# appyjain21/pilottai

Hardware: AMD Instinct MI355X
Metric: completed agent-tasks/sec (whole node) + p50 task latency, 64 concurrent workers (higher is better)
Workload: dtype bf16

## Files before the change

csrc/ops/gemm_stream.hip:

```cpp
#include "common.h"
#include "packed_epi.h"

#include <algorithm>
#include <type_traits>

namespace pa {
namespace sg {

using pk::EP_PLAIN;
using pk::EP_SILU;
using pk::EP_RESID;
using pk::EP_ROPEPERM;
using pk::EP_ROPEKV;
using pk::store_quad;

struct Args {
  bf16* y;
  const bf16* x;
  const bf16* wp;
  const bf16* resid;
  float* ws;
  int* counters;
  int* err;
  int M, N, K, ldx, ldy, ldr;
  int S, RG, G;
  int KSW;
  int epi;
  float eps;
  const float* ss_in;
  float* ss_out;
  float* ss_zero;
  bf16* q_out;
  bf16* k_cache;
  bf16* v_cache;
  const int* positions;
  const int* slots;
  const float* cos_sin;
  int H, KV;
  int rel;
  unsigned long long* stamps;
};

typedef __attribute__((address_space(1))) int gi32;

template <int N>
__device__ __forceinline__ void wait_lgkm() {
  static_assert(N >= 0 && N < 16, "lgkmcnt is 4 bits");
  __builtin_amdgcn_s_waitcnt(0xF | (7 << 4) | (N << 8) | (3 << 14));
}

__device__ __forceinline__ void raw_barrier() {
  asm volatile("" ::: "memory");
  __builtin_amdgcn_s_barrier();
  asm volatile("" ::: "memory");
}

__device__ __forceinline__ void group_barrier(int* arrive, int n, int* err, int rel) {
  __syncthreads();
  if (threadIdx.x == 0) {
    if (rel) {
      __builtin_amdgcn_fence(__ATOMIC_RELEASE, "agent");
      asm volatile("s_waitcnt vmcnt(0)" ::: "memory");
    }
    const int tk = __hip_atomic_fetch_add((gi32*)arrive, 1, __ATOMIC_RELAXED, __HIP_MEMORY_SCOPE_AGENT);
    if (tk != n - 1) {
      const unsigned long long t0 = __builtin_amdgcn_s_memrealtime();
      while (__hip_atomic_load((gi32*)arrive, __ATOMIC_RELAXED, __HIP_MEMORY_SCOPE_AGENT) < n) {
        __builtin_amdgcn_s_sleep(1);
        if (__builtin_amdgcn_s_memrealtime() - t0 > 100000000ull) {
          __hip_atomic_store((gi32*)err, 1, __ATOMIC_RELAXED, __HIP_MEMORY_SCOPE_AGENT);
          break;
        }
      }
    }
    __builtin_amdgcn_fence(__ATOMIC_ACQUIRE, "agent");
    asm volatile("s_waitcnt vmcnt(0)" ::: "memory");
  }
  __syncthreads();
}

template <int EPI>
__device__ __forceinline__ float epi_quad(const Args& A, int m, int tile, int cq, f32x4 v, f32x4 v2) {
  return store_quad<EPI>(A, m, tile, cq, v, v2);
}

struct Pre {
  float rs;
  bf16x4 rv;
  f32x4 c, sn;
  int slot;
};

__device__ __forceinline__ Pre preload(const Args& A, int m, int tile, int cq) {
  Pre p;
  p.rs = 1.f;
  p.slot = -1;
  p.c = f32x4{1.f, 1.f, 1.f, 1.f};
  p.sn = f32x4{0.f, 0.f, 0.f, 0.f};
  if (m >= A.M) return p;
  if (A.ss_in) p.rs = rsqrtf(A.ss_in[m] * (1.f / (float)A.K) + A.eps);
  if (A.epi == EP_RESID) {
    p.rv = *reinterpret_cast<const bf16x4*>(A.resid + (size_t)m * A.ldr + tile * 16 + cq);
  } else if (A.epi == EP_ROPEKV) {
    const int hh = tile >> 3;
    const int d = 16 * ((tile & 7) >> 1) + cq;
    if (hh < A.H + A.KV) {
      const float* cs = A.cos_sin + (size_t)A.positions[m] * 128;
      p.c = *reinterpret_cast<const f32x4*>(cs + d);
      p.sn = *reinterpret_cast<const f32x4*>(cs + 64 + d);
    }
    if (hh >= A.H) p.slot = A.slots[m];
  }
  return p;
}

__device__ __forceinline__ float epi_pre(const Args& A, int m, int tile, int cq, f32x4 v, f32x4 v2, const Pre& p) {
  if (A.epi == EP_SILU) return store_quad<EP_SILU>(A, m, tile, cq, v, v2);
  if (A.epi == EP_PLAIN) return store_quad<EP_PLAIN>(A, m, tile, cq, v, v2);
  if (A.epi == EP_ROPEPERM) return store_quad<EP_ROPEPERM>(A, m, tile, cq, v, v2);
  if (A.epi == EP_RESID) {
    bf16x4 o;
    float sq = 0.f;
#pragma unroll
    for (int r = 0; r < 4; ++r) {
      o[r] = (bf16)(v[r] + (float)p.rv[r]);
      const float f = (float)o[r];
      sq = fmaf(f, f, sq);
    }
    *reinterpret_cast<bf16x4*>(A.y + (size_t)m * A.ldy + tile * 16 + cq) = o;
    return sq;
  }
  const int hh = tile >> 3;
  const int d = 16 * ((tile & 7) >> 1) + cq;
  f32x4 o1 = v, o2 = v2;
  if (hh < A.H + A.KV) {
    o1 = v * p.c - v2 * p.sn;
    o2 = v2 * p.c + v * p.sn;
  }
  bf16x4 b1, b2;
#pragma unroll
  for (int r = 0; r < 4; ++r) {
    b1[r] = (bf16)o1[r];
    b2[r] = (bf16)o2[r];
  }
  if (hh < A.H) {
    bf16* dst = A.q_out + ((size_t)m * A.H + hh) * 128;
    *reinterpret_cast<bf16x4*>(dst + d) = b1;
    *reinterpret_cast<bf16x4*>(dst + d + 64) = b2;
  } else if (p.slot >= 0) {
    const int blk = p.slot >> 4, off = p.slot & 15;
    if (hh < A.H + A.KV) {
      bf16* page = A.k_cache + ((size_t)blk * A.KV + (hh - A.H)) * 128 * 16;
      *reinterpret_cast<bf16x4*>(page + ((size_t)(d >> 3) * 16 + off) * 8 + (d & 7)) = b1;
      *reinterpret_cast<bf16x4*>(page + ((size_t)((d + 64) >> 3) * 16 + off) * 8 + (d & 7)) = b2;
    } else {
      bf16* page = A.v_cache + ((size_t)blk * A.KV + (hh - A.H - A.KV)) * 128 * 16 + off;
#pragma unroll
      for (int r = 0; r < 4; ++r) {
        page[(size_t)(d + r) * 16] = b1[r];
        page[(size_t)(d + 64 + r) * 16] = b2[r];
      }
    }
  }
  return 0.f;
}

template <int MG, int TPW, int WT, int WK, int D>
__global__ __launch_bounds__(WT * WK * 64) void stream_gemm_kernel(const Args A) {
  constexpr int W = WT * WK, NTH = W * 64;
  constexpr int MT = 16 * MG;
  constexpr int CT = WT * TPW;
  constexpr int KW = 2, KC = 2 * WK;
  constexpr int XCH = WK * MT * 128;
  constexpr int XU = WK * MT * 8;
  constexpr int LX = (XU + NTH - 1) / NTH;
  static_assert(D == 2 || D == 4 || D == 8 || D == 16, "even ring depth (LDS slot = chunk & 1)");
  __shared__ __attribute__((aligned(1024))) char smem[2 * XCH + MT * 4 + 16];
  float* rsq = reinterpret_cast<float*>(smem + 2 * XCH);

  const int lane = threadIdx.x & 63;
  const int wid = __builtin_amdgcn_readfirstlane(threadIdx.x >> 6);
  const int wt = wid % WT, wk = wid / WT;
  const int nwg = gridDim.x, bid = blockIdx.x;
  const int q8 = nwg >> 3, r8 = nwg & 7, xcd = bid & 7;
  const int work = (xcd < r8 ? xcd * (q8 + 1) : r8 * (q8 + 1) + (xcd - r8) * q8) + (bid >> 3);
  const int rg = work % A.RG;
  const int s = (work / A.RG) % A.S;
  const int grp = work / (A.RG * A.S);
  const int gid = grp * A.RG + rg;
  const int row0 = rg * MT;
  const int t0 = grp * CT;
  const int KS = A.K >> 5;
  const int kb0 = s * A.KSW;
  const int nch = A.KSW / KC;
  const int rot = (A.rel & 2) ? (work * 5) % nch : 0;

  auto stamp = [&](int i) {
    if (A.stamps && threadIdx.x == 0) A.stamps[(size_t)bid * 8 + i] = __builtin_amdgcn_s_memrealtime();
  };
  stamp(0);
  if (A.ss_zero && bid == 0)
    for (int i = threadIdx.x; i < A.M; i += NTH) A.ss_zero[i] = 0.f;
  for (int i = threadIdx.x; i < MT; i += NTH) rsq[i] = 0.f;

  const bf16x8* wsrc[TPW];
#pragma unroll
  for (int j = 0; j < TPW; ++j)
    wsrc[j] = reinterpret_cast<const bf16x8*>(A.wp + ((size_t)(t0 + wt * TPW + j) * KS + kb0 + wk * KW) * 512) + lane;
  const bf16* xsrc[LX];
  int xdst[LX];
#pragma unroll
  for (int i = 0; i < LX; ++i) {
    const int e = (threadIdx.x + i * NTH) % XU;
    const int h = e / (MT * 8), r = (e >> 3) % MT, u = e & 7;
    const int gr = min(row0 + r, A.M - 1);
    xsrc[i] = A.x + (size_t)gr * A.ldx + kb0 * 32 + h * 64 + u * 8;
    xdst[i] = h * MT * 128 + r * 128 + ((u ^ ((r >> 1) & 7)) << 4);
  }

  bf16x8 wr[D][KW][TPW];
  bf16x8 xr[D][LX];
  f32x4 acc[MG][TPW];
#pragma unroll
  for (int i = 0; i < MG; ++i)
#pragma unroll
    for (int j = 0; j < TPW; ++j) acc[i][j] = f32x4{0.f, 0.f, 0.f, 0.f};

  auto issue = [&](int c0, int d) {
    const int c = rot ? (c0 + rot) % nch : c0;
    __builtin_amdgcn_sched_barrier(0);
#pragma unroll
    for (int i = 0; i < LX; ++i) xr[d][i] = *reinterpret_cast<const bf16x8*>(xsrc[i] + (size_t)c * KC * 32);
#pragma unroll
    for (int i = 0; i < KW; ++i)
#pragma unroll
      for (int j = 0; j < TPW; ++j) wr[d][i][j] = __builtin_nontemporal_load(wsrc[j] + (size_t)(c * KC + i) * 64);
    __builtin_amdgcn_sched_barrier(0);
  };
  auto consume = [&](int d, int slot) {
    char* st = smem + slot * XCH;
#pragma unroll
    for (int i = 0; i < LX; ++i) *reinterpret_cast<bf16x8*>(st + xdst[i]) = xr[d][i];
    wait_lgkm<0>();
    raw_barrier();
#pragma unroll
    for (int i = 0; i < KW; ++i) {
      const int kk = wk * KW + i;
      const int hb = (kk >> 1) * MT * 128, ks = kk & 1;
      bf16x8 xf[MG];
#pragma unroll
      for (int mg = 0; mg < MG; ++mg) {
        const int row = mg * 16 + (lane & 15);
        const int u = 4 * ks + (lane >> 4);
        xf[mg] = *reinterpret_cast<const bf16x8*>(st + hb + row * 128 + ((u ^ ((row >> 1) & 7)) << 4));
      }
#pragma unroll
      for (int mg = 0; mg < MG; ++mg)
#pragma unroll
        for (int j = 0; j < TPW; ++j)
          acc[mg][j] = __builtin_amdgcn_mfma_f32_16x16x32_bf16(wr[d][i][j], xf[mg], acc[mg][j], 0, 0, 0);
    }
  };

#pragma unroll
  for (int d = 0; d < D; ++d) issue(d, d);
  int c = 0;
  for (; c + D < nch; c += D) {
#pragma unroll
    for (int d = 0; d < D; ++d) {
      consume(d, d & 1);
      if (c == 0 && d == 0) stamp(1);
      issue(c + d + D, d);
    }
  }
#pragma unroll
  for (int d = 0; d < D; ++d) {
    consume(d, d & 1);
    if (c == 0 && d == 0) stamp(1);
  }
  stamp(2);

  const bool pair = A.epi == EP_SILU || A.epi == EP_ROPEKV;
  const float inv_k = 1.f / (float)A.K;
  const int g = lane >> 4, cl = lane & 15;
  auto epi_any = [&](int m, int tile, f32x4 v, f32x4 v2) -> float {
    switch (A.epi) {
      case EP_PLAIN: return epi_quad<EP_PLAIN>(A, m, tile, 4 * g, v, v2);
      case EP_SILU: return epi_quad<EP_SILU>(A, m, tile, 4 * g, v, v2);
      case EP_RESID: return epi_quad<EP_RESID>(A, m, tile, 4 * g, v, v2);
      case EP_ROPEPERM: return epi_quad<EP_ROPEPERM>(A, m, tile, 4 * g, v, v2);
      default: return epi_quad<EP_ROPEKV>(A, m, tile, 4 * g, v, v2);
    }
  };
  auto row_stat = [&](int mg, int m, float sq) {
    sq += __shfl_xor(sq, 16, 64);
    sq += __shfl_xor(sq, 32, 64);
    if (g == 0 && m < A.M) atomicAdd(rsq + mg * 16 + cl, sq);
  };
  auto flush_row_stats = [&]() {
    __syncthreads();
    if (A.ss_out)
      for (int i = threadIdx.x; i < MT; i += NTH) {
        const float v = rsq[i];
        if (v != 0.f && row0 + i < A.M) atomicAdd(A.ss_out + row0 + i, v);
      }
  };

  if (A.S * WK == 1 && (!pair || TPW % 2 == 0)) {
#pragma unroll
    for (int mg = 0; mg < MG; ++mg) {
      const int m = row0 + mg * 16 + cl;
      float sq = 0.f;
      if (m < A.M) {
        const float rs = A.ss_in ? rsqrtf(A.ss_in[m] * inv_k + A.eps) : 1.f;
        if (pair) {
#pragma unroll
          for (int j = 0; j + 1 < TPW; j += 2) epi_any(m, t0 + wt * TPW + j, acc[mg][j] * rs, acc[mg][j + 1] * rs);
        } else {
#pragma unroll
          for (int j = 0; j < TPW; ++j) sq += epi_any(m, t0 + wt * TPW + j, acc[mg][j] * rs, acc[mg][j]);
        }
      }
      if (A.ss_out) row_stat(mg, m, sq);
    }
    flush_row_stats();
    stamp(3);
    stamp(4);
    return;
  }

  const int TU = pair ? CT / 2 : CT;
  const int U = TU * MG;
  const int u0 = s + A.S * wid;
  Pre pre0{};
  if (u0 < U) {
    const int tl = pair ? 2 * (u0 / MG) : u0 / MG;
    pre0 = preload(A, row0 + (u0 % MG) * 16 + cl, t0 + tl, 4 * g);
  }

  const int SV = A.S * WK;
  float* gslab = A.ws + (size_t)gid * SV * CT * MG * 256;
  {
    const __amdgpu_buffer_rsrc_t rs =
        __builtin_amdgcn_make_buffer_rsrc(gslab, 0, SV * CT * MG * 1024, 0x00020000);
    const int sv = s * WK + wk;
#pragma unroll
    for (int j = 0; j < TPW; ++j)
#pragma unroll
      for (int mg = 0; mg < MG; ++mg) {
        const int f = (wt * TPW + j) * MG + mg;
        __builtin_amdgcn_raw_buffer_store_b128(__builtin_bit_cast(u32x4, acc[mg][j]), rs,
                                               ((sv * CT * MG + f) * 64 + lane) * 16, 0, 16);
      }
  }
  asm volatile("s_waitcnt vmcnt(0)" ::: "memory");
  int* ctr = A.counters + 2 * gid;
  group_barrier(ctr, A.S, A.err, A.rel & 1);
  stamp(3);

  const __amdgpu_buffer_rsrc_t ra = __builtin_amdgcn_make_buffer_rsrc(gslab, 0, SV * CT * MG * 1024, 0x00020000);
  for (int u = s + A.S * wid; u < U; u += A.S * W) {
    const int tu = u / MG, mg = u % MG;
    const int tl = pair ? 2 * tu : tu;
    const int f = tl * MG + mg;
    f32x4 v = f32x4{0.f, 0.f, 0.f, 0.f}, v2 = f32x4{0.f, 0.f, 0.f, 0.f};
    auto gather = [&](auto two) {
      constexpr bool TWO = decltype(two)::value;
      for (int p0 = 0; p0 < SV; p0 += 8) {
        f32x4 ta[8], tb[8];
#pragma unroll
        for (int q = 0; q < 8; ++q) {
          const int p = min(p0 + q, SV - 1);
          ta[q] = __builtin_bit_cast(f32x4, __builtin_amdgcn_raw_buffer_load_b128(ra, ((p * CT * MG + f) * 64 + lane) * 16, 0, 16));
          if constexpr (TWO)
            tb[q] = __builtin_bit_cast(
                f32x4, __builtin_amdgcn_raw_buffer_load_b128(ra, ((p * CT * MG + f + MG) * 64 + lane) * 16, 0, 16));
        }
#pragma unroll
        for (int q = 0; q < 8; ++q) {
          const float keep = p0 + q < SV ? 1.f : 0.f;
          v += ta[q] * keep;
          if constexpr (TWO) v2 += tb[q] * keep;
        }
      }
    };
    if (pair) gather(std::true_type{});
    else gather(std::false_type{});
    const int m = row0 + mg * 16 + cl;
    float sq = 0.f;
    if (m < A.M) {
      if (u == u0) {
        sq = epi_pre(A, m, t0 + tl, 4 * g, v * pre0.rs, v2 * pre0.rs, pre0);
      } else {
        const float rs = A.ss_in ? rsqrtf(A.ss_in[m] * inv_k + A.eps) : 1.f;
        sq = epi_any(m, t0 + tl, v * rs, v2 * rs);
      }
    }
    if (A.ss_out) row_stat(mg, m, sq);
  }
  flush_row_stats();
  stamp(4);
  if (threadIdx.x == 0) {
    const int left = __hip_atomic_fetch_add((gi32*)(ctr + 1), 1, __ATOMIC_RELAXED, __HIP_MEMORY_SCOPE_AGENT);
    if (left == A.S - 1) {
      __hip_atomic_store((gi32*)ctr, 0, __ATOMIC_RELAXED, __HIP_MEMORY_SCOPE_AGENT);
      __hip_atomic_store((gi32*)(ctr + 1), 0, __ATOMIC_RELAXED, __HIP_MEMORY_SCOPE_AGENT);
    }
  }
}

struct Shape {
  int tpw, wt, wk;
};
static const Shape kShapes[] = {
    {1, 4, 1}, {2, 4, 1}, {3, 4, 1}, {4, 4, 1}, {1, 4, 2}, {2, 2, 2}, {3, 2, 2},
    {1, 6, 1}, {2, 6, 1}, {2, 7, 1}, {2, 8, 1}, {1, 8, 1},
};

template <int MG, int TPW, int WT, int WK>
static bool launch_d(const Args& a, int D, int grid, hipStream_t st) {
  switch (D) {
    case 2: hipLaunchKernelGGL((stream_gemm_kernel<MG, TPW, WT, WK, 2>), dim3(grid), dim3(WT * WK * 64), 0, st, a); return true;
    case 4: hipLaunchKernelGGL((stream_gemm_kernel<MG, TPW, WT, WK, 4>), dim3(grid), dim3(WT * WK * 64), 0, st, a); return true;
    case 8: hipLaunchKernelGGL((stream_gemm_kernel<MG, TPW, WT, WK, 8>), dim3(grid), dim3(WT * WK * 64), 0, st, a); return true;
    case 16: hipLaunchKernelGGL((stream_gemm_kernel<MG, TPW, WT, WK, 16>), dim3(grid), dim3(WT * WK * 64), 0, st, a); return true;
    default: return false;
  }
}

template <int MG>
static bool launch_mg(const Args& a, int tpw, int wt, int wk, int D, int grid, hipStream_t st) {
#define PA_SG(T_, W_, K_) \
  if (tpw == T_ && wt == W_ && wk == K_) return launch_d<MG, T_, W_, K_>(a, D, grid, st);
  PA_SG(1, 4, 1) PA_SG(2, 4, 1) PA_SG(3, 4, 1) PA_SG(4, 4, 1) PA_SG(1, 4, 2) PA_SG(2, 2, 2) PA_SG(3, 2, 2)
  PA_SG(1, 6, 1) PA_SG(2, 6, 1) PA_SG(2, 7, 1) PA_SG(2, 8, 1) PA_SG(1, 8, 1)
#undef PA_SG
  return false;
}

struct Plan {
  int mg, rg, tpw, wt, wk, S, D;
};

static int num_cus() {
  static int n = 0;
  if (n == 0) {
    int dev = 0, v = 0;
    if (hipGetDevice(&dev) == hipSuccess && hipDeviceGetAttribute(&v, hipDeviceAttributeMultiprocessorCount, dev) == hipSuccess && v > 0)
      n = v;
    else
      n = 256;
  }
  return n;
}

static bool plan_ok(const Plan& p, int M, int N, int K, int epi) {
  const int tiles = N / 16, KS = K / 32;
  const int CT = p.tpw * p.wt;
  if (p.mg != 2 && p.mg != 4 && p.mg != 8) return false;
  if (p.rg < 1 || 16 * p.mg * p.rg < M || 16 * p.mg * (p.rg - 1) >= M) return false;
  if (tiles % CT) return false;
  if ((epi == EP_SILU || epi == EP_ROPEKV) && CT % 2) return false;
  if (p.S < 1 || KS % p.S) return false;
  const int KC = 2 * p.wk;
  const int ksw = KS / p.S;
  if (ksw % KC) return false;
  const int nch = ksw / KC;
  if (nch < p.D || nch % p.D) return false;
  if (p.S > 1 && (tiles / CT) * p.rg * p.S > num_cus()) return false;
  return true;
}

static Plan plan_default(int M, int N, int K, int epi) {
  Plan p{};
  p.mg = M <= 32 ? 2 : (M <= 64 ? 4 : 8);
  p.rg = (M + 16 * p.mg - 1) / (16 * p.mg);
  const int tiles = N / 16;
  const bool two = p.rg > 1;
  p.wk = 1;
  p.D = 4;
  if (tiles == 1792) {
    p.tpw = 2; p.wt = 7; p.S = two ? 1 : 2;
  } else if (K >= 8192) {
    p.tpw = 2; p.wt = 4; p.S = two ? 4 : 8;
  } else if (tiles == 384) {
    if (two) { p.tpw = 3; p.wt = 4; p.S = 4; }
    else { p.tpw = 3; p.wt = 2; p.wk = 2; p.S = 4; }
  } else if (tiles == 256) {
    if (two) { p.tpw = 2; p.wt = 4; p.S = 4; }
    else { p.tpw = 1; p.wt = 4; p.wk = 2; p.S = 4; }
  } else if (tiles % 16 == 0 && tiles >= 4096) {
    p.tpw = 4; p.wt = 4; p.S = 1;
  } else {
    p.tpw = 1; p.wt = 4; p.S = 1; p.D = 2;
  }
  if (!plan_ok(p, M, N, K, epi)) {
    p.tpw = 1; p.wt = 4; p.wk = 1; p.S = 1; p.D = 2;
  }
  return p;
}

}
}

extern "C" long long pa_stream_gemm_ws_floats(int M, int N, int K, int mg, int rg, int tpw, int wt, int wk, int S) {
  (void)M; (void)K;
  const long long CT = (long long)tpw * wt, G = N / 16 / CT;
  return G * rg * S * wk * CT * mg * 256;
}

extern "C" void pa_stream_gemm_plan(int M, int N, int K, int epi, int* plan) {
  const pa::sg::Plan p = pa::sg::plan_default(M, N, K, epi);
  plan[0] = p.mg; plan[1] = p.rg; plan[2] = p.tpw; plan[3] = p.wt; plan[4] = p.wk; plan[5] = p.S; plan[6] = p.D;
}

extern "C" int pa_stream_gemm(void* y, const void* x, const void* wp, const void* resid, float* ws,
                              long long ws_floats, int* counters, int n_counters, int* err, int M, int N, int K,
                              int ldx, int ldy, int ldr, int epi, const float* ss_in, float* ss_out, float* ss_zero,
                              float eps, const int* plan, void* q_out, void* k_cache, void* v_cache,
                              const int* positions, const int* slots, const float* cos_sin, int H, int KV, int rel,
                              unsigned long long* stamps, hipStream_t st) {
  using namespace pa::sg;
  if (M <= 0) return 0;
  if (M > 256 || K % 64 != 0 || N % 16 != 0 || epi < 0 || epi > 4) return 1;
  if (epi == EP_RESID && !resid) return 1;
  if (ss_out && epi != EP_RESID) return 1;
  if (epi == EP_ROPEKV && (!q_out || !k_cache || !v_cache || !positions || !slots || !cos_sin ||
                           N != (H + 2 * KV) * 128))
    return 1;
  Plan p = plan_default(M, N, K, epi);
  if (plan && plan[0] > 0 && plan[1] > 0 && plan[2] > 0 && plan[3] > 0 && plan[4] > 0 && plan[5] > 0 && plan[6] > 0)
    p = Plan{plan[0], plan[1], plan[2], plan[3], plan[4], plan[5], plan[6]};
  if (!plan_ok(p, M, N, K, epi)) return 1;
  const int CT = p.tpw * p.wt;
  const int G = N / 16 / CT;
  const int groups = G * p.rg;
  if (!ws || !counters || !err || n_counters < 2 * groups) return 1;
  const bool direct = p.S * p.wk == 1 && (!(epi == EP_SILU || epi == EP_ROPEKV) || p.tpw % 2 == 0);
  if (!direct && pa_stream_gemm_ws_floats(M, N, K, p.mg, p.rg, p.tpw, p.wt, p.wk, p.S) > ws_floats) return 1;
  const int grid = groups * p.S;
  Args a{(pa::bf16*)y, (const pa::bf16*)x, (const pa::bf16*)wp, (const pa::bf16*)resid, ws, counters, err,
         M, N, K, ldx, ldy, ldr, p.S, p.rg, G, K / 32 / p.S, epi, eps, ss_in, ss_out, ss_zero,
         (pa::bf16*)q_out, (pa::bf16*)k_cache, (pa::bf16*)v_cache, positions, slots, cos_sin, H, KV, rel,
         stamps};
  bool ok = false;
  switch (p.mg) {
    case 2: ok = launch_mg<2>(a, p.tpw, p.wt, p.wk, p.D, grid, st); break;
    case 4: ok = launch_mg<4>(a, p.tpw, p.wt, p.wk, p.D, grid, st); break;
    case 8: ok = launch_mg<8>(a, p.tpw, p.wt, p.wk, p.D, grid, st); break;
    default: ok = false;
  }
  if (!ok) return 1;
  return (int)hipGetLastError() == 0 ? 0 : -2;
}
```

pilottai_amd/models/llama.py:

```python
from __future__ import annotations

import math
import os
from dataclasses import dataclass, field
from typing import Dict, List, Optional

import torch
import torch.nn.functional as F

from pilottai_amd import ops
from pilottai_amd.ops import reference as ref
from pilottai_amd.parallel.comm import TPGroup


@dataclass
class LlamaConfig:
    name: str = "llama-3-8b"
    vocab_size: int = 128256
    hidden_size: int = 4096
    intermediate_size: int = 14336
    num_layers: int = 32
    num_heads: int = 32
    num_kv_heads: int = 8
    head_dim: int = 128
    rope_theta: float = 500000.0
    rope_scaling: Optional[dict] = None
    rms_eps: float = 1e-5
    max_position: int = 8192
    tie_embeddings: bool = False
    init_std: float = 0.02

    @property
    def gqa_group(self) -> int:
        return self.num_heads // self.num_kv_heads

    def num_params(self) -> int:
        d, f, v = self.hidden_size, self.intermediate_size, self.vocab_size
        qkv = d * (self.num_heads + 2 * self.num_kv_heads) * self.head_dim
        per_layer = qkv + self.num_heads * self.head_dim * d + 3 * d * f + 2 * d
        return self.num_layers * per_layer + v * d * (1 if self.tie_embeddings else 2) + d


PRESETS: Dict[str, LlamaConfig] = {
    "llama-3-8b": LlamaConfig(),
    "llama-3-70b": LlamaConfig(name="llama-3-70b", hidden_size=8192, intermediate_size=28672,
                               num_layers=80, num_heads=64, num_kv_heads=8),
    "llama-3.1-8b": LlamaConfig(name="llama-3.1-8b", max_position=131072,
                                rope_scaling={"factor": 8.0, "low_freq_factor": 1.0,
                                              "high_freq_factor": 4.0,
                                              "original_max_position_embeddings": 8192}),
    "tiny": LlamaConfig(name="tiny", hidden_size=512, intermediate_size=1024, num_layers=2,
                        num_heads=4, num_kv_heads=1, max_position=4096),
    "tiny-gqa4": LlamaConfig(name="tiny-gqa4", hidden_size=1024, intermediate_size=2048,
                             num_layers=2, num_heads=8, num_kv_heads=2, max_position=4096),
    "tiny-kv8": LlamaConfig(name="tiny-kv8", hidden_size=1024, intermediate_size=2048, num_layers=2,
                            num_heads=16, num_kv_heads=8, max_position=4096),
    "llama-3-8b-2l": LlamaConfig(name="llama-3-8b-2l", num_layers=2, max_position=4096),
    "llama-3-70b-1l": LlamaConfig(name="llama-3-70b-1l", hidden_size=8192, intermediate_size=28672,
                                  num_layers=1, num_heads=64, num_kv_heads=8, max_position=4096),
    "llama-3-70b-2l": LlamaConfig(name="llama-3-70b-2l", hidden_size=8192, intermediate_size=28672,
                                  num_layers=2, num_heads=64, num_kv_heads=8, max_position=4096),
}


def get_config(name_or_cfg) -> LlamaConfig:
    if isinstance(name_or_cfg, LlamaConfig):
        return name_or_cfg
    key = str(name_or_cfg).lower()
    if key not in PRESETS:
        raise ValueError(f"unknown model {name_or_cfg!r}; known: {sorted(PRESETS)}")
    return PRESETS[key]


@dataclass
class StepMeta:
    input_ids: torch.Tensor
    positions: torch.Tensor
    slots: torch.Tensor
    q_start: torch.Tensor
    q_len: torch.Tensor
    ctx_len: torch.Tensor
    block_table: torch.Tensor
    items: torch.Tensor
    n_items: torch.Tensor
    att_counters: torch.Tensor
    logit_rows: torch.Tensor
    num_seqs: int = 0
    part_size: Optional[torch.Tensor] = None


class KVCache:

    def __init__(self, num_layers: int, num_blocks: int, kv_heads: int, device, dtype=torch.bfloat16,
                 block_size: int = 16):
        self.num_blocks = num_blocks
        self.block_size = block_size
        self.k = torch.zeros(num_layers, num_blocks, kv_heads, 16, block_size, 8, dtype=dtype, device=device)
        self.v = torch.zeros(num_layers, num_blocks, kv_heads, 128, block_size, dtype=dtype, device=device)

    @staticmethod
    def bytes_per_block(num_layers: int, kv_heads: int, block_size: int = 16) -> int:
        return 2 * num_layers * kv_heads * block_size * 128 * 2


DENSE_KINDS = ("wqkv", "wo", "w13", "w2")


class LlamaModel:
    DECODE_FUSED_MAX_T = 16
    MID_MAX_T = 256
    PREFILL_MAX_T = 1 << 30
    PF_MIDRANGE = frozenset({"gate_up"})
    DEC_QKV_MAX_T = 0
    ATT_DECODE_WAVES = int(os.environ.get("PILOTTAI_ATT_DECODE_WAVES", "8"))
    ATT_MID_WAVES = int(os.environ.get("PILOTTAI_ATT_MID_WAVES", "4"))
    PF_CFG = {
        "qkv": [(80, "mid", {}), (1280, "pf", {"bn": 128, "variant": 3}),
                (2048, "pf", {"bn": 192, "variant": 3}), (3840, "pf", {"bn": 256, "variant": 3}),
                (1 << 30, "pf", {"bn": 192, "variant": 3})],
        "o": [(128, "mid", {}), (1 << 30, "pf", {"bn": 128, "variant": 3})],
        "gate_up": [(128, "mid", {}), (256, "pf", {"bn": 128, "variant": 3}),
                    (1 << 30, "pf", {"bn": 256, "variant": 3})],
        "down": [(128, "mid", {}), (512, "pf", {"bn": 128, "variant": 3}),
                 (1 << 30, "pf", {"bn": 256, "variant": 3})],
    }
    STREAM_CFG: Dict[str, list] = {
        "qkv": [(32, (1, 1, 4, 1, 2, 4))],
        "o": [(64, (1, 1, 4, 1, 4, 4)), (128, (1, 1, 4, 1, 4, 2))],
        "down": [(32, (1, 1, 4, 1, 4, 4)), (128, (1, 2, 4, 1, 8, 2)), (256, (2, 2, 8, 1, 7, 2))],
    }
    STREAM_NK: Dict[str, tuple] = {"qkv": (6144, 4096), "o": (4096, 4096), "gate_up": (28672, 4096),
                                   "down": (4096, 14336), "lm_head": (128256, 4096)}
    LM_HEAD_STREAM: list = [(32, (1, 3, 4, 1, 1, 2)), (64, (1, 4, 4, 1, 1, 2)), (128, (1, 2, 8, 1, 1, 2))]
    MID_CFG = {
        "qkv": [(32, 1, 2, 2), (64, 1, 2, 1), (128, 2, 2, 1), (256, 4, 2, 1), (1 << 30, 4, 4, 1)],
        "o": [(32, 1, 2, 4), (64, 1, 2, 2), (128, 2, 2, 2), (256, 2, 2, 1), (1 << 30, 4, 2, 1)],
        "gate_up": [(32, 1, 4, 1), (64, 2, 4, 1), (128, 4, 4, 1), (256, 8, 4, 1), (1 << 30, 8, 4, 1)],
        "down": [(32, 1, 2, 4), (64, 2, 2, 4), (128, 2, 2, 2), (256, 4, 2, 2), (1 << 30, 4, 4, 2)],
    }

    def __init__(self, cfg: LlamaConfig, device, dtype=torch.bfloat16, tp: Optional[TPGroup] = None,
                 seed: int = 0, weights_path: Optional[str] = None, decode_pack: Optional[bool] = None,
                 keep_dense: Optional[bool] = None, weight_quant: Optional[str] = None, fp8_decode: bool = True):
        self.cfg = cfg
        self.device = torch.device(device)
        self.dtype = dtype
        self.tp = tp or TPGroup.single()
        if weight_quant not in (None, "fp8"):
            raise ValueError(f"unknown weight_quant {weight_quant!r} (None or 'fp8')")
        if weight_quant and self.tp.size > 1:
            raise ValueError("weight_quant='fp8' needs tensor-parallel size 1: per-channel scales of "
                             "row-parallel shards are not designed yet")
        if weight_quant and decode_pack is False:
            raise ValueError("weight_quant='fp8' lives on the packed weight copies: it cannot be combined "
                             "with decode_pack=False (EngineConfig.decode_fused=False)")
        self.weight_quant = weight_quant
        self.fp8_decode = bool(fp8_decode) and weight_quant == "fp8"
        ov = os.environ.get("PILOTTAI_ROUTING_JSON")
        if ov:
            import json

            for table, rows in json.loads(ov).items():
                if table == "PF_MIDRANGE":
                    self.PF_MIDRANGE = frozenset(rows)
                    continue
                if table not in ("STREAM_CFG", "MID_CFG", "PF_CFG"):
                    raise ValueError(f"PILOTTAI_ROUTING_JSON: unknown table {table!r}")
                merged = dict(getattr(self, table))
                for kind, r in rows.items():
                    merged[kind] = [tuple(x) if table == "MID_CFG" else
                                    (x[0], tuple(x[1])) if table == "STREAM_CFG" else (x[0], x[1], dict(x[2]))
                                    for x in r]
                setattr(self, table, merged)
        ts = self.tp.size
        if cfg.num_heads % ts or cfg.num_kv_heads % ts or cfg.intermediate_size % ts or cfg.vocab_size % ts:
            raise ValueError(f"{cfg.name} is not divisible by tensor-parallel size {ts}")
        self.h_local = cfg.num_heads // ts
        self.kv_local = cfg.num_kv_heads // ts
        self.f_local = cfg.intermediate_size // ts
        self.v_local = cfg.vocab_size // ts
        self.vocab_offset = self.tp.rank * self.v_local
        self.scale = 1.0 / math.sqrt(cfg.head_dim)
        self.cos_sin = ref.rope_cos_sin(cfg.max_position, cfg.head_dim, cfg.rope_theta,
                                        cfg.rope_scaling).to(self.device)
        if weights_path:
            self._load_hf(weights_path)
        else:
            self._init_random(seed)
        self.decode_packed = False
        self.keep_dense = (self.device.type != "cuda") if keep_dense is None else bool(keep_dense)
        if decode_pack is None:
            decode_pack = self._pack_fits()
        if weight_quant:
            self._check_quant_fits(decode_pack)
        if decode_pack:
            self._pack_decode_weights()

    def _pack_fits(self) -> bool:
        if self.device.type != "cuda":
            return True
        total = torch.cuda.get_device_properties(self.device).total_memory
        extra = self._fp8_copy_bytes() if self.fp8_decode else 0
        if self.keep_dense:
            return 2 * self.weight_bytes() + extra <= 0.45 * total
        return self.weight_bytes() + extra <= 0.7 * total

    def _fp8_copy_bytes(self) -> int:
        n = 0
        for L in self.layers:
            for k in DENSE_KINDS:
                w = L[k]
                n += w.numel() + 4 * w.shape[0]
        return n

    def _check_quant_fits(self, decode_pack: bool):
        if decode_pack or self.device.type != "cuda":
            return
        total = torch.cuda.get_device_properties(self.device).total_memory
        base, extra = self.weight_bytes(), (self._fp8_copy_bytes() if self.fp8_decode else 0)
        hint = (": build the model with fp8_decode=False (the same quantised model on the bf16 decode kernels)"
                if self.fp8_decode else "")
        raise ValueError(f"weight_quant={self.weight_quant!r}: {base / 1e9:.2f} GB of bf16 weights"
                         f"{' (kept row-major copy doubles them)' if self.keep_dense else ''} + "
                         f"{extra / 1e9:.2f} GB of FP8 decode copies do not fit beside the KV cache on a "
                         f"{total / 1e9:.0f} GB device{hint}")

    def _pack_decode_weights(self):
        for L in self.layers:
            if self.weight_quant == "fp8":
                self._pack_layer_fp8(L)
            else:
                L["wqkv_p"] = ops.pack_decode_qkv_rope(L["wqkv"] * L["ln1"][None, :])
                L["wo_p"] = ops.pack_decode_weight(L["wo"])
                L["w13_p"] = ops.pack_decode_gate_up(L["w13"] * L["ln2"][None, :])
                L["w2_p"] = ops.pack_decode_weight(L["w2"])
            if not self.keep_dense:
                for k in DENSE_KINDS:
                    del L[k]
        self.lm_head_p = ops.pack_decode_weight(self.lm_head)
        if not self.keep_dense and self.lm_head is not self.embed and self.lm_head.shape[0] % 256 == 0:
            self.lm_head = None
        if self.device.type == "cuda":
            ops.decode_workspace(self.device)
            ops.mid_workspace(self.device)
            ops.prefill_workspace(self.device)
            ops.stream_workspace(self.device)
        self._ss = torch.zeros(2, 1 << 15, dtype=torch.float32, device=self.device)
        self.decode_packed = True

    def _pack_layer_fp8(self, L: Dict[str, torch.Tensor]):
        plan = (("wqkv", "ln1", ops.pack_decode_qkv_rope, ops.pack_decode_qkv_rope_fp8),
                ("wo", None, ops.pack_decode_weight, ops.pack_decode_weight_fp8),
                ("w13", "ln2", ops.pack_decode_gate_up, ops.pack_decode_gate_up_fp8),
                ("w2", None, ops.pack_decode_weight, ops.pack_decode_weight_fp8))
        for kind, ln, pack, pack8 in plan:
            w = L[kind] * L[ln][None, :] if ln else L[kind]
            q, s = ops.quantize_fp8_rows(w)
            deq = ops.dequantize_fp8_rows(q, s, self.dtype)
            del w
            L[kind + "_p"] = pack(deq)
            if self.fp8_decode:
                L[kind + "_p8"], L[kind + "_s8"] = pack8((q, s))
            if self.keep_dense:
                L[kind] = (deq.float() / L[ln].float()[None, :]).to(self.dtype) if ln else deq
            del q, s, deq

    def dense(self, L: Dict[str, torch.Tensor], kind: str) -> torch.Tensor:
        w = L.get(kind)
        if w is not None:
            return w
        if kind == "wqkv":
            return (ops.unpack_decode_qkv_rope(L["wqkv_p"]).float() / L["ln1"].float()[None, :]).to(self.dtype)
        if kind == "w13":
            return (ops.unpack_decode_gate_up(L["w13_p"]).float() / L["ln2"].float()[None, :]).to(self.dtype)
        return ops.unpack_decode_weight(L[{"wo": "wo_p", "w2": "w2_p"}[kind]])

    def dense_lm_head(self) -> torch.Tensor:
        return self.lm_head if self.lm_head is not None else ops.unpack_decode_weight(self.lm_head_p)

    def _dense_needed(self, T: int) -> bool:
        return not self.decode_packed or T > max(self.MID_MAX_T, self.PREFILL_MAX_T)

    def _init_random(self, seed: int):
        cfg, dev, dt = self.cfg, self.device, self.dtype
        C = cfg.num_kv_heads
        ts, r = self.tp.size, self.tp.rank
        if C % ts:
            raise ValueError(f"TP size {ts} must divide num_kv_heads={C}")
        mine = range(r * C // ts, (r + 1) * C // ts)
        std, d, hd = cfg.init_std, cfg.hidden_size, cfg.head_dim

        def chunk(tag: int, j: int, *shape):
            g = torch.Generator(device=dev)
            g.manual_seed((seed * 1_000_003 + tag * 7919 + j) & 0x7FFFFFFF)
            t = torch.empty(*shape, dtype=dt, device=dev)
            t.normal_(0.0, std, generator=g)
            return t

        def rows(tag, total_rows, cols):
            return torch.cat([chunk(tag, j, total_rows // C, cols) for j in mine], 0)

        def colsplit(tag, rows_, total_cols):
            return torch.cat([chunk(tag, j, rows_, total_cols // C) for j in mine], 1)

        self.embed = rows(1, cfg.vocab_size, d)
        self.layers: List[Dict[str, torch.Tensor]] = []
        for li in range(cfg.num_layers):
            t = 100 + 10 * li
            q = rows(t + 0, cfg.num_heads * hd, d)
            k = rows(t + 1, cfg.num_kv_heads * hd, d)
            v = rows(t + 2, cfg.num_kv_heads * hd, d)
            gate = rows(t + 4, cfg.intermediate_size, d)
            up = rows(t + 5, cfg.intermediate_size, d)
            self.layers.append({
                "ln1": torch.ones(d, dtype=dt, device=dev),
                "wqkv": torch.cat([q, k, v], 0),
                "wo": colsplit(t + 3, d, cfg.num_heads * hd),
                "ln2": torch.ones(d, dtype=dt, device=dev),
                "w13": torch.cat([gate, up], 0),
                "w2": colsplit(t + 6, d, cfg.intermediate_size),
            })
            del q, k, v, gate, up
        self.norm = torch.ones(d, dtype=dt, device=dev)
        self.lm_head = self.embed if cfg.tie_embeddings else rows(2, cfg.vocab_size, d)

    def _load_hf(self, path: str):
        from safetensors import safe_open

        cfg, dev, dt = self.cfg, self.device, self.dtype
        files = sorted(f for f in os.listdir(path) if f.endswith(".safetensors"))
        tensors: Dict[str, torch.Tensor] = {}
        for f in files:
            with safe_open(os.path.join(path, f), framework="pt") as fh:
                for k in fh.keys():
                    tensors[k] = fh.get_tensor(k)
        r, ts, hd = self.tp.rank, self.tp.size, cfg.head_dim

        def rows(t, n):
            return t.chunk(ts, dim=0)[r] if ts > 1 else t

        def cols(t):
            return t.chunk(ts, dim=1)[r] if ts > 1 else t

        def get(k):
            return tensors[k].to(dt)

        self.embed = rows(get("model.embed_tokens.weight"), 0).to(dev)
        self.layers = []
        for i in range(cfg.num_layers):
            p = f"model.layers.{i}."
            q = rows(get(p + "self_attn.q_proj.weight"), 0)
            k = rows(get(p + "self_attn.k_proj.weight"), 0)
            v = rows(get(p + "self_attn.v_proj.weight"), 0)
            gate = rows(get(p + "mlp.gate_proj.weight"), 0)
            up = rows(get(p + "mlp.up_proj.weight"), 0)
            self.layers.append({
                "ln1": get(p + "input_layernorm.weight").to(dev),
                "wqkv": torch.cat([q, k, v], 0).contiguous().to(dev),
                "wo": cols(get(p + "self_attn.o_proj.weight")).contiguous().to(dev),
                "ln2": get(p + "post_attention_layernorm.weight").to(dev),
                "w13": torch.cat([gate, up], 0).contiguous().to(dev),
                "w2": cols(get(p + "mlp.down_proj.weight")).contiguous().to(dev),
            })
            del q, k, v, gate, up
        self.norm = get("model.norm.weight").to(dev)
        if "lm_head.weight" in tensors and not cfg.tie_embeddings:
            self.lm_head = rows(get("lm_head.weight"), 0).contiguous().to(dev)
        else:
            self.lm_head = self.embed
        _ = hd

    def weight_bytes(self) -> int:
        n = self.embed.numel() + self.norm.numel()
        if self.lm_head is not None and self.lm_head is not self.embed:
            n += self.lm_head.numel()
        if getattr(self, "lm_head_p", None) is not None:
            n += self.lm_head_p.numel()
        n *= self.embed.element_size()
        for L in self.layers:
            n += sum(t.numel() * t.element_size() for t in L.values())
        return n

    def _embed(self, ids: torch.Tensor) -> torch.Tensor:
        if self.tp.size == 1:
            return F.embedding(ids, self.embed)
        local = ids - self.vocab_offset
        ok = (local >= 0) & (local < self.v_local)
        h = F.embedding(local.clamp(0, self.v_local - 1), self.embed) * ok.unsqueeze(-1).to(self.dtype)
        self.tp.all_reduce(h)
        return h

    def forward(self, meta: StepMeta, kv: KVCache, num_tokens: int, num_logit_rows: int,
                part_o: torch.Tensor, part_ml: torch.Tensor, embed=None) -> torch.Tensor:
        cfg = self.cfg
        T = num_tokens
        if self.decode_packed and T <= self.DECODE_FUSED_MAX_T:
            return self._forward_decode(meta, kv, T, num_logit_rows, part_o, part_ml, embed)
        if self.decode_packed and (T <= self.MID_MAX_T or T <= self.PREFILL_MAX_T):
            return self._forward_mid(meta, kv, T, num_logit_rows, part_o, part_ml, embed)
        H, KVh, hd = self.h_local, self.kv_local, cfg.head_dim
        if not self.keep_dense and self.decode_packed:
            raise RuntimeError(f"a {T}-token step needs the row-major weights, which were freed after packing: "
                               "build the model with keep_dense=True (EngineConfig.keep_dense) to run such steps "
                               "on the library GEMMs")
        ids = meta.input_ids[:T].long() if self.device.type == "cpu" else meta.input_ids[:T]
        h = self._embed(ids)
        resid = h
        x = ops.rmsnorm(h, self.layers[0]["ln1"], cfg.rms_eps)
        for li, L in enumerate(self.layers):
            qkv = ops.linear(x, L["wqkv"], "qkv")
            q = torch.empty(T, H, hd, dtype=self.dtype, device=self.device)
            ops.rope_cache(q, kv.k[li], kv.v[li], qkv, meta.positions, meta.slots, self.cos_sin, H, KVh)
            attn = torch.empty(T, H, hd, dtype=self.dtype, device=self.device)
            ops.paged_attention(attn, part_o, part_ml, q, kv.k[li], kv.v[li], meta.items, meta.n_items,
                                meta.att_counters, meta.q_start, meta.q_len, meta.ctx_len,
                                meta.block_table, self.scale, num_seqs=meta.num_seqs, part_size=meta.part_size)
            o = ops.linear(attn.view(T, H * hd), L["wo"], "o")
            if self.tp.size > 1:
                self.tp.all_reduce(o)
            x = ops.fused_add_rmsnorm(resid, o, L["ln2"], cfg.rms_eps)
            gu = ops.linear(x, L["w13"], "gate_up")
            a = ops.silu_mul(gu)
            d = ops.linear(a, L["w2"], "down")
            if self.tp.size > 1:
                self.tp.all_reduce(d)
            nxt = self.layers[li + 1]["ln1"] if li + 1 < len(self.layers) else self.norm
            x = ops.fused_add_rmsnorm(resid, d, nxt, cfg.rms_eps)
        if embed is not None:
            self._pool_embed(x, T, embed)
        rows = meta.logit_rows[:num_logit_rows]
        rows = rows.long() if self.device.type == "cpu" else rows
        xs = x.index_select(0, rows)
        return ops.linear(xs, self.lm_head, "lm_head")

    def _forward_decode(self, meta: StepMeta, kv: KVCache, T: int, num_logit_rows: int,
                        part_o: torch.Tensor, part_ml: torch.Tensor, embed=None) -> torch.Tensor:
        cfg = self.cfg
        H, KVh, hd = self.h_local, self.kv_local, cfg.head_dim
        eps = cfg.rms_eps
        tp = self.tp.size > 1
        ids = meta.input_ids[:T].long() if self.device.type == "cpu" else meta.input_ids[:T]
        h = self._embed(ids)
        if not h.is_contiguous():
            h = h.contiguous()
        for li, L in enumerate(self.layers):
            q = torch.empty(T, H, hd, dtype=self.dtype, device=self.device)
            f8 = "wqkv_p8" in L
            if f8:
                ops.decode_qkv_rope_fp8(h, L["wqkv_p8"], L["wqkv_s8"], eps, q, kv.k[li], kv.v[li], meta.positions,
                                        meta.slots, self.cos_sin, H, KVh)
            else:
                ops.decode_qkv_rope(h, L["wqkv_p"], eps, q, kv.k[li], kv.v[li], meta.positions, meta.slots,
                                    self.cos_sin, H, KVh)
            attn = torch.empty(T, H, hd, dtype=self.dtype, device=self.device)
            ops.paged_attention(attn, part_o, part_ml, q, kv.k[li], kv.v[li], meta.items, meta.n_items,
                                meta.att_counters, meta.q_start, meta.q_len, meta.ctx_len,
                                meta.block_table, self.scale, num_seqs=meta.num_seqs, part_size=meta.part_size,
                                waves=self.ATT_DECODE_WAVES)
            a2 = attn.view(T, H * hd)
            if f8:
                ops.decode_gemm_fp8(a2, L["wo_p8"], L["wo_s8"], "resid", resid=h, out=h)
                a = ops.decode_gemm_fp8(h, L["w13_p8"], L["w13_s8"], "silu", norm=True, eps=eps)
                ops.decode_gemm_fp8(a, L["w2_p8"], L["w2_s8"], "resid", resid=h, out=h, **self._down_cfg(T))
                continue
            if tp:
                self.tp.all_reduce_add(ops.decode_gemm(a2, L["wo_p"], "plain"), h)
            else:
                ops.decode_gemm(a2, L["wo_p"], "resid", resid=h, out=h)
            a = ops.decode_gemm(h, L["w13_p"], "silu", norm=True, eps=eps)
            if tp:
                self.tp.all_reduce_add(ops.decode_gemm(a, L["w2_p"], "plain"), h)
            else:
                ops.decode_gemm(a, L["w2_p"], "resid", resid=h, out=h, **self._down_cfg(T))
        if embed is not None:
            self._pool_embed(ops.rmsnorm(h, self.norm, eps), T, embed)
        rows = meta.logit_rows[:num_logit_rows]
        rows = rows.long() if self.device.type == "cpu" else rows
        xs = ops.rmsnorm(h.index_select(0, rows), self.norm, eps)
        return ops.decode_gemm(xs, self.lm_head_p, "plain")

    @staticmethod
    def _down_cfg(T: int) -> dict:
        return {"nt": 1, "waves": 8}

    @staticmethod
    def _pool_embed(hn: torch.Tensor, T: int, embed):
        rows, pool = embed[:2]
        pool[-1].zero_()
        pool.index_add_(0, rows[:T].long(), hn[:T].float())
        if len(embed) > 2:
            n_seg, segs, span_pool = embed[2][:3]
            ops.kernels.span_pool(hn[:T], n_seg, segs, span_pool)

    def _mid_cfg(self, kind: str, T: int) -> dict:
        for mmax, fm, fn, S in self.MID_CFG[kind]:
            if T <= mmax:
                return {"fm": fm, "fn": fn, "splits": S}
        return {}

    @staticmethod
    def _stream_plan(M: int, shape) -> tuple:
        rg0, tpw, wt, wk, S, D = (int(v) for v in shape)
        for rg in sorted(range(1, 17), key=lambda r: (abs(r - rg0), r)):
            need = -(-M // (16 * rg))
            mg = next((m for m in (2, 4, 8) if m >= need), 0)
            if mg and 16 * mg * (rg - 1) < M:
                return (mg, rg, tpw, wt, wk, S, D)
        raise ValueError(f"no stream plan for M={M} with shape {shape}")

    @staticmethod
    def _stream_plan_ok(plan, M: int, N: int, K: int, pair: bool) -> bool:
        mg, rg, tpw, wt, wk, S, D = plan
        tiles, KS, CT = N // 16, K // 32, tpw * wt
        if N % 16 or K % 64 or tiles % CT or (pair and CT % 2) or KS % S or (KS // S) % (2 * wk):
            return False
        nch = KS // S // (2 * wk)
        if nch < D or nch % D or 16 * mg * rg < M or 16 * mg * (rg - 1) >= M:
            return False
        grid = tiles // CT * rg * S
        if S > 1 and grid > 256:
            return False
        from pilottai_amd.ops import kernels

        direct = S * wk == 1 and (not pair or tpw % 2 == 0)
        return direct or (tiles // CT) * rg * S * wk * CT * mg * 256 <= kernels.STREAM_WS_FLOATS

    def _stream_for(self, kind: str, T: int, N: int, K: int, rows, pair: bool = False):
        nk = self.STREAM_NK.get(kind)
        if nk is not None and tuple(nk) != (N, K):
            return None
        for mmax, shape in rows:
            if T <= mmax:
                try:
                    plan = self._stream_plan(T, shape)
                except ValueError:
                    return None
                return plan if self._stream_plan_ok(plan, T, N, K, pair) else None
        return None

    def _proj_path(self, kind: str, T: int, N: int = 0, K: int = 0):
        if T <= self.MID_MAX_T and N:
            plan = self._stream_for(kind, T, N, K, self.STREAM_CFG.get(kind, ()),
                                    pair=kind in ("qkv", "gate_up"))
            if plan is not None:
                return "stream", {"plan": plan}
        if self.device.type == "cuda" and (T > self.MID_MAX_T or kind in self.PF_MIDRANGE):
            for mmax, path, cfg in self.PF_CFG[kind]:
                if T <= mmax:
                    if path != "pf":
                        return path, self._mid_cfg(kind, T) | dict(cfg)
                    cfg = dict(cfg)
                    if cfg.get("bn") == 192 and N % 192:
                        cfg["bn"] = 256
                    return path, cfg
        return "mid", self._mid_cfg(kind, T)

    def _gemm(self, kind: str, T: int, x, wp, epi: str, ordered: bool = False, **kw):
        path, cfg = self._proj_path(kind, T, wp.shape[0] * 16, wp.shape[1] * 32)
        if ordered and path == "pf":
            cfg = dict(cfg, splits=1)
        fn = {"pf": ops.prefill_gemm, "stream": ops.stream_gemm}.get(path, ops.mid_gemm)
        return fn(x, wp, epi, **cfg, **kw)

    def _qkv_rope(self, T: int, x, wp, eps, q, k_cache, v_cache, meta, ss_in, ordered: bool = False):
        H, KVh = self.h_local, self.kv_local
        if T <= min(self.DEC_QKV_MAX_T, 64) and self.device.type == "cuda":
            return ops.decode_qkv_rope(x, wp, eps, q, k_cache, v_cache, meta.positions, meta.slots, self.cos_sin,
                                       H, KVh)
        path, cfg = self._proj_path("qkv", T, wp.shape[0] * 16, wp.shape[1] * 32)
        if ordered and path == "pf":
            cfg = dict(cfg, splits=1)
        fn = {"pf": ops.prefill_qkv_rope, "stream": ops.stream_qkv_rope}.get(path, ops.mid_qkv_rope)
        return fn(x, wp, eps, q, k_cache, v_cache, meta.positions, meta.slots, self.cos_sin, H, KVh,
                  ss_in=ss_in, **cfg)

    def _forward_mid(self, meta: StepMeta, kv: KVCache, T: int, num_logit_rows: int,
                     part_o: torch.Tensor, part_ml: torch.Tensor, embed=None) -> torch.Tensor:
        cfg = self.cfg
        H, KVh, hd = self.h_local, self.kv_local, cfg.head_dim
        eps = cfg.rms_eps
        tp = self.tp.size > 1
        ids = meta.input_ids[:T].long() if self.device.type == "cpu" else meta.input_ids[:T]
        h = self._embed(ids)
        if not h.is_contiguous():
            h = h.contiguous()
        ss_a, ss_b = self._ss[0, :T], self._ss[1, :T]
        ordered = embed is not None and len(embed) > 2 and not tp and (len(embed[2]) < 4 or bool(embed[2][3]))
        ops.row_sumsq(h, out=ss_a)
        ss_b.zero_()
        for li, L in enumerate(self.layers):
            q = torch.empty(T, H, hd, dtype=self.dtype, device=self.device)
            self._qkv_rope(T, h, L["wqkv_p"], eps, q, kv.k[li], kv.v[li], meta, ss_a, ordered)
            attn = torch.empty(T, H, hd, dtype=self.dtype, device=self.device)
            ops.paged_attention(attn, part_o, part_ml, q, kv.k[li], kv.v[li], meta.items, meta.n_items,
                                meta.att_counters, meta.q_start, meta.q_len, meta.ctx_len,
                                meta.block_table, self.scale, num_seqs=meta.num_seqs, part_size=meta.part_size,
                                waves=self.ATT_MID_WAVES)
            a2 = attn.view(T, H * hd)
            if tp:
                self.tp.all_reduce_add(self._gemm("o", T, a2, L["wo_p"], "plain"), h, ss=ss_b, ss_zero=ss_a)
            elif ordered:
                self._gemm("o", T, a2, L["wo_p"], "resid", ordered=True, resid=h, out=h)
                ops.row_sumsq(h, out=ss_b)
            else:
                self._gemm("o", T, a2, L["wo_p"], "resid", resid=h, out=h, ss_out=ss_b, ss_zero=ss_a)
            a = self._gemm("gate_up", T, h, L["w13_p"], "silu", ordered=ordered, norm=True, eps=eps, ss_in=ss_b)
            if tp:
                self.tp.all_reduce_add(self._gemm("down", T, a, L["w2_p"], "plain"), h, ss=ss_a, ss_zero=ss_b)
            elif ordered:
                self._gemm("down", T, a, L["w2_p"], "resid", ordered=True, resid=h, out=h)
                ops.row_sumsq(h, out=ss_a)
            else:
                self._gemm("down", T, a, L["w2_p"], "resid", resid=h, out=h, ss_out=ss_a, ss_zero=ss_b)
        if embed is not None:
            self._pool_embed(ops.rmsnorm(h, self.norm, eps), T, embed)
        rows = meta.logit_rows[:num_logit_rows]
        rows = rows.long() if self.device.type == "cpu" else rows
        xs = ops.rmsnorm(h.index_select(0, rows), self.norm, eps)
        return self._lm_head(xs, num_logit_rows)

    def _lm_head(self, xs, n: int):
        if n > self.DECODE_FUSED_MAX_T:
            wp = self.lm_head_p
            plan = self._stream_for("lm_head", n, wp.shape[0] * 16, wp.shape[1] * 32, self.LM_HEAD_STREAM)
            if plan is not None:
                return ops.stream_gemm(xs, wp, "plain", plan=plan)
        if n <= 32:
            return ops.decode_gemm(xs, self.lm_head_p, "plain")
        if self.lm_head is None:
            return ops.prefill_gemm(xs, self.lm_head_p, "plain")
        return ops.linear(xs, self.lm_head, "lm_head")

    @torch.no_grad()
    def reference_logits(self, token_ids: List[int]) -> torch.Tensor:
        assert self.tp.size == 1
        cfg = self.cfg
        T = len(token_ids)
        ids = torch.tensor(token_ids, device=self.device)
        h = F.embedding(ids, self.embed).float()
        pos = torch.arange(T, device=self.device)
        H, KVh, hd = self.h_local, self.kv_local, cfg.head_dim
        mask = torch.full((T, T), float("-inf"), device=self.device).triu(1)
        for L0 in self.layers:
            L = {k: self.dense(L0, k) for k in DENSE_KINDS}
            L["ln1"], L["ln2"] = L0["ln1"], L0["ln2"]
            x = ref.rmsnorm(h.to(self.dtype), L["ln1"], cfg.rms_eps).float()
            qkv = (x.to(self.dtype).float() @ L["wqkv"].float().T).to(self.dtype)
            q = ref.apply_rope(qkv[:, :H * hd].view(T, H, hd), pos, self.cos_sin)
            k = ref.apply_rope(qkv[:, H * hd:(H + KVh) * hd].view(T, KVh, hd), pos, self.cos_sin)
            v = qkv[:, (H + KVh) * hd:].view(T, KVh, hd)
            G = H // KVh
            kh = k.float().repeat_interleave(G, 1).permute(1, 0, 2)
            vh = v.float().repeat_interleave(G, 1).permute(1, 0, 2)
            s = (q.float().permute(1, 0, 2) @ kh.transpose(1, 2)) * self.scale + mask
            o = (torch.softmax(s, -1) @ vh).permute(1, 0, 2).reshape(T, H * hd).to(self.dtype)
            h = (h.to(self.dtype).float() + (o.float() @ L["wo"].float().T).to(self.dtype).float())
            x = ref.rmsnorm(h.to(self.dtype), L["ln2"], cfg.rms_eps)
            gu = (x.float() @ L["w13"].float().T).to(self.dtype)
            a = ref.silu_mul(gu)
            h = (h.to(self.dtype).float() + (a.float() @ L["w2"].float().T).to(self.dtype).float())
        x = ref.rmsnorm(h.to(self.dtype), self.norm, cfg.rms_eps)
        return (x.float() @ self.dense_lm_head().float().T)

    @torch.no_grad()
    def hidden_states(self, batch: List[List[int]], pooling: str = "mean") -> torch.Tensor:
        assert self.tp.size == 1, "hidden_states runs on a TP=1 model"
        cfg, dev, dt = self.cfg, self.device, self.dtype
        B = len(batch)
        T = max(1, max(len(s) for s in batch))
        ids = torch.zeros(B, T, dtype=torch.long, device=dev)
        valid = torch.zeros(B, T, dtype=torch.bool, device=dev)
        for i, s in enumerate(batch):
            if s:
                ids[i, :len(s)] = torch.tensor(s, device=dev)
                valid[i, :len(s)] = True
        H, KVh, hd = self.h_local, self.kv_local, cfg.head_dim
        pos = torch.arange(T, device=dev)
        cs = self.cos_sin[:T]
        cos, sin = cs[:, : hd // 2].to(dt), cs[:, hd // 2:].to(dt)

        def rope(x):
            x1, x2 = x[..., : hd // 2], x[..., hd // 2:]
            c, s = cos[None, :, None, :], sin[None, :, None, :]
            return torch.cat([x1 * c - x2 * s, x2 * c + x1 * s], dim=-1)

        h = F.embedding(ids, self.embed)
        for L0 in self.layers:
            L = {k: self.dense(L0, k) for k in DENSE_KINDS}
            x = F.rms_norm(h, (cfg.hidden_size,), L0["ln1"], cfg.rms_eps)
            qkv = F.linear(x, L["wqkv"])
            q = rope(qkv[..., : H * hd].view(B, T, H, hd))
            k = rope(qkv[..., H * hd:(H + KVh) * hd].view(B, T, KVh, hd))
            v = qkv[..., (H + KVh) * hd:].view(B, T, KVh, hd)
            o = F.scaled_dot_product_attention(q.transpose(1, 2), k.transpose(1, 2), v.transpose(1, 2),
                                               is_causal=True, enable_gqa=True, scale=self.scale)
            h = h + F.linear(o.transpose(1, 2).reshape(B, T, H * hd), L["wo"])
            x = F.rms_norm(h, (cfg.hidden_size,), L0["ln2"], cfg.rms_eps)
            gu = F.linear(x, L["w13"])
            g, u = gu.chunk(2, dim=-1)
            h = h + F.linear(F.silu(g) * u, L["w2"])
        x = F.rms_norm(h, (cfg.hidden_size,), self.norm, cfg.rms_eps).float()
        if pooling == "last":
            last = torch.tensor([max(1, len(s)) - 1 for s in batch], device=dev)
            return x[torch.arange(B, device=dev), last]
        w = valid.unsqueeze(-1).float()
        return (x * w).sum(1) / w.sum(1).clamp_min(1.0)
```

Before: 43.66.

## Add 12/16-row-group stream GEMM tiles for 129-192 row down projection

Extends the streaming GEMM kernel to support MG of 12 and 16, so a single workgroup covers up to 256 rows. The LDS activation fragments are loaded in half-groups to limit register pressure, and dead row groups are skipped in the epilogue and split-K reduction. A new down-projection config routes 129-192 token batches to a single row group, so each weight tile is streamed once instead of twice. This trades higher VGPR use and shallower prefetch rings (D<=4) for the halved weight traffic.

```diff
diff --git a/csrc/ops/gemm_stream.hip b/csrc/ops/gemm_stream.hip
--- a/csrc/ops/gemm_stream.hip
+++ b/csrc/ops/gemm_stream.hip
@@ -175,6 +175,8 @@
   constexpr int XU = WK * MT * 8;
   constexpr int LX = (XU + NTH - 1) / NTH;
   static_assert(D == 2 || D == 4 || D == 8 || D == 16, "even ring depth (LDS slot = chunk & 1)");
+  static_assert(MG <= 8 || (MG % 2 == 0 && MG <= 16 && D <= 4), "129-256 rows per workgroup: shallow rings only");
+  constexpr int XG = MG > 8 ? MG / 2 : MG;
   __shared__ __attribute__((aligned(1024))) char smem[2 * XCH + MT * 4 + 16];
   float* rsq = reinterpret_cast<float*>(smem + 2 * XCH);
 
@@ -189,6 +191,7 @@
   const int grp = work / (A.RG * A.S);
   const int gid = grp * A.RG + rg;
   const int row0 = rg * MT;
+  const int live = MG > 8 ? min(MG, (A.M - row0 + 15) >> 4) : MG;
   const int t0 = grp * CT;
   const int KS = A.K >> 5;
   const int kb0 = s * A.KSW;
@@ -247,18 +250,21 @@
     for (int i = 0; i < KW; ++i) {
       const int kk = wk * KW + i;
       const int hb = (kk >> 1) * MT * 128, ks = kk & 1;
-      bf16x8 xf[MG];
-#pragma unroll
-      for (int mg = 0; mg < MG; ++mg) {
-        const int row = mg * 16 + (lane & 15);
-        const int u = 4 * ks + (lane >> 4);
-        xf[mg] = *reinterpret_cast<const bf16x8*>(st + hb + row * 128 + ((u ^ ((row >> 1) & 7)) << 4));
-      }
-#pragma unroll
-      for (int mg = 0; mg < MG; ++mg)
-#pragma unroll
-        for (int j = 0; j < TPW; ++j)
-          acc[mg][j] = __builtin_amdgcn_mfma_f32_16x16x32_bf16(wr[d][i][j], xf[mg], acc[mg][j], 0, 0, 0);
+#pragma unroll
+      for (int m0 = 0; m0 < MG; m0 += XG) {
+        bf16x8 xf[XG];
+#pragma unroll
+        for (int mg = 0; mg < XG; ++mg) {
+          const int row = (m0 + mg) * 16 + (lane & 15);
+          const int u = 4 * ks + (lane >> 4);
+          xf[mg] = *reinterpret_cast<const bf16x8*>(st + hb + row * 128 + ((u ^ ((row >> 1) & 7)) << 4));
+        }
+#pragma unroll
+        for (int mg = 0; mg < XG; ++mg)
+#pragma unroll
+          for (int j = 0; j < TPW; ++j)
+            acc[m0 + mg][j] = __builtin_amdgcn_mfma_f32_16x16x32_bf16(wr[d][i][j], xf[mg], acc[m0 + mg][j], 0, 0, 0);
+      }
     }
   };
 
@@ -309,6 +315,7 @@
   if (A.S * WK == 1 && (!pair || TPW % 2 == 0)) {
 #pragma unroll
     for (int mg = 0; mg < MG; ++mg) {
+      if (MG > 8 && mg >= live) continue;
       const int m = row0 + mg * 16 + cl;
       float sq = 0.f;
       if (m < A.M) {
@@ -348,6 +355,7 @@
     for (int j = 0; j < TPW; ++j)
 #pragma unroll
       for (int mg = 0; mg < MG; ++mg) {
+        if (MG > 8 && mg >= live) continue;
         const int f = (wt * TPW + j) * MG + mg;
         __builtin_amdgcn_raw_buffer_store_b128(__builtin_bit_cast(u32x4, acc[mg][j]), rs,
                                                ((sv * CT * MG + f) * 64 + lane) * 16, 0, 16);
@@ -361,6 +369,7 @@
   const __amdgpu_buffer_rsrc_t ra = __builtin_amdgcn_make_buffer_rsrc(gslab, 0, SV * CT * MG * 1024, 0x00020000);
   for (int u = s + A.S * wid; u < U; u += A.S * W) {
     const int tu = u / MG, mg = u % MG;
+    if (MG > 8 && mg >= live) continue;
     const int tl = pair ? 2 * tu : tu;
     const int f = tl * MG + mg;
     f32x4 v = f32x4{0.f, 0.f, 0.f, 0.f}, v2 = f32x4{0.f, 0.f, 0.f, 0.f};
@@ -422,10 +431,16 @@
   switch (D) {
     case 2: hipLaunchKernelGGL((stream_gemm_kernel<MG, TPW, WT, WK, 2>), dim3(grid), dim3(WT * WK * 64), 0, st, a); return true;
     case 4: hipLaunchKernelGGL((stream_gemm_kernel<MG, TPW, WT, WK, 4>), dim3(grid), dim3(WT * WK * 64), 0, st, a); return true;
-    case 8: hipLaunchKernelGGL((stream_gemm_kernel<MG, TPW, WT, WK, 8>), dim3(grid), dim3(WT * WK * 64), 0, st, a); return true;
-    case 16: hipLaunchKernelGGL((stream_gemm_kernel<MG, TPW, WT, WK, 16>), dim3(grid), dim3(WT * WK * 64), 0, st, a); return true;
-    default: return false;
-  }
+    default: break;
+  }
+  if constexpr (MG <= 8) {
+    switch (D) {
+      case 8: hipLaunchKernelGGL((stream_gemm_kernel<MG, TPW, WT, WK, 8>), dim3(grid), dim3(WT * WK * 64), 0, st, a); return true;
+      case 16: hipLaunchKernelGGL((stream_gemm_kernel<MG, TPW, WT, WK, 16>), dim3(grid), dim3(WT * WK * 64), 0, st, a); return true;
+      default: break;
+    }
+  }
+  return false;
 }
 
 template <int MG>
@@ -457,7 +472,8 @@
 static bool plan_ok(const Plan& p, int M, int N, int K, int epi) {
   const int tiles = N / 16, KS = K / 32;
   const int CT = p.tpw * p.wt;
-  if (p.mg != 2 && p.mg != 4 && p.mg != 8) return false;
+  if (p.mg != 2 && p.mg != 4 && p.mg != 8 && p.mg != 12 && p.mg != 16) return false;
+  if (p.mg > 8 && p.D > 4) return false;
   if (p.rg < 1 || 16 * p.mg * p.rg < M || 16 * p.mg * (p.rg - 1) >= M) return false;
   if (tiles % CT) return false;
   if ((epi == EP_SILU || epi == EP_ROPEKV) && CT % 2) return false;
@@ -476,6 +492,10 @@
   p.mg = M <= 32 ? 2 : (M <= 64 ? 4 : 8);
   p.rg = (M + 16 * p.mg - 1) / (16 * p.mg);
   const int tiles = N / 16;
+  if (M > 128 && M <= 192 && K >= 8192 && tiles != 1792) {
+    const Plan one{12, 1, 1, 8, 1, 7, 2};
+    if (plan_ok(one, M, N, K, epi)) return one;
+  }
   const bool two = p.rg > 1;
   p.wk = 1;
   p.D = 4;
@@ -548,6 +568,8 @@
     case 2: ok = launch_mg<2>(a, p.tpw, p.wt, p.wk, p.D, grid, st); break;
     case 4: ok = launch_mg<4>(a, p.tpw, p.wt, p.wk, p.D, grid, st); break;
     case 8: ok = launch_mg<8>(a, p.tpw, p.wt, p.wk, p.D, grid, st); break;
+    case 12: ok = launch_mg<12>(a, p.tpw, p.wt, p.wk, p.D, grid, st); break;
+    case 16: ok = launch_mg<16>(a, p.tpw, p.wt, p.wk, p.D, grid, st); break;
     default: ok = false;
   }
   if (!ok) return 1;
diff --git a/pilottai_amd/models/llama.py b/pilottai_amd/models/llama.py
--- a/pilottai_amd/models/llama.py
+++ b/pilottai_amd/models/llama.py
@@ -127,7 +127,8 @@
     STREAM_CFG: Dict[str, list] = {
         "qkv": [(32, (1, 1, 4, 1, 2, 4))],
         "o": [(64, (1, 1, 4, 1, 4, 4)), (128, (1, 1, 4, 1, 4, 2))],
-        "down": [(32, (1, 1, 4, 1, 4, 4)), (128, (1, 2, 4, 1, 8, 2)), (256, (2, 2, 8, 1, 7, 2))],
+        "down": [(32, (1, 1, 4, 1, 4, 4)), (128, (1, 2, 4, 1, 8, 2)), (192, (1, 1, 8, 1, 7, 2)),
+                 (256, (2, 2, 8, 1, 7, 2))],
     }
     STREAM_NK: Dict[str, tuple] = {"qkv": (6144, 4096), "o": (4096, 4096), "gate_up": (28672, 4096),
                                    "down": (4096, 14336), "lm_head": (128256, 4096)}
@@ -501,9 +502,10 @@
     @staticmethod
     def _stream_plan(M: int, shape) -> tuple:
         rg0, tpw, wt, wk, S, D = (int(v) for v in shape)
+        mgs = (2, 4, 8, 12, 16) if D <= 4 else (2, 4, 8)
         for rg in sorted(range(1, 17), key=lambda r: (abs(r - rg0), r)):
             need = -(-M // (16 * rg))
-            mg = next((m for m in (2, 4, 8) if m >= need), 0)
+            mg = next((m for m in mgs if m >= need), 0)
             if mg and 16 * mg * (rg - 1) < M:
                 return (mg, rg, tpw, wt, wk, S, D)
         raise ValueError(f"no stream plan for M={M} with shape {shape}")
@@ -513,6 +515,8 @@
         mg, rg, tpw, wt, wk, S, D = plan
         tiles, KS, CT = N // 16, K // 32, tpw * wt
         if N % 16 or K % 64 or tiles % CT or (pair and CT % 2) or KS % S or (KS // S) % (2 * wk):
+            return False
+        if mg not in (2, 4, 8, 12, 16) or (mg > 8 and D > 4):
             return False
         nch = KS // S // (2 * wk)
         if nch < D or nch % D or 16 * mg * rg < M or 16 * mg * (rg - 1) >= M:
```

Measured after the change: 43.87, median of 5. Within noise of the previous version (+0.5%).
